# dblanm/gnn-manip

Hardware: AMD Instinct MI355X
Metric: rollout steps/sec (N particles, 10 MP steps, hidden=128) (higher is better)
Workload: dtype f32; 1 GPU; north_star target: N=100k dense synthetic scene, conn_r=0.015, max_neighbours=20, hidden=128, 10 MP steps; n_particles=100000, hidden=128, edges_last_step=1966056, k_steps=6, candidates_per_gpu=1, parallelism=candidate-parallel x1

## Files before the change

gnn_manip_amd/csrc/hedge.hip:

```cpp
#include <type_traits>
#include "common.h"
#include "mlp.h"
#include "hedge.h"
#include "hmlp.h"
#include "hmma_dev.h"
#include "blocks_dev.h"

namespace gm {

namespace {

constexpr int H = 128;
constexpr int BE = 32;
constexpr int SYS_THREADS = 768;
static_assert(BE == kBlockEdges, "block tables and the systolic kernels agree on the block size");
#ifdef HEDGE_STAMPS
__device__ unsigned long long g_sys_stamps[3 * 32 * 8 + 32];
#define SYS_STAMP(tick, slot)                                                                                         \
    do {                                                                                                              \
        if (blockIdx.x == 0 && jb == 0 && lane0 == 0 && (tick) >= 16 && (tick) < 48) {                                \
            g_sys_stamps[(role * 32 + (tick) - 16) * 8 + (slot)] = __builtin_readcyclecounter();                     \
            if (role == 0 && (slot) == 0) g_sys_stamps[3 * 32 * 8 + (tick) - 16] = __builtin_amdgcn_s_memrealtime(); \
        }                                                                                                             \
    } while (0)
// ... 141 lines not shown
}
__device__ __forceinline__ float sum_of_halves(float v) {
    const auto r = __builtin_amdgcn_permlane32_swap(__float_as_uint(v), __float_as_uint(v), false, false);
    return __uint_as_float(r[0]) + __uint_as_float(r[1]);
}

template <int R>
__device__ __forceinline__ void scan3_t(float& ya, float& yb, float& yc, float yprev, unsigned cont) {
    asm volatile("s_bfe_i32 exec_lo, %4, %5\n\ts_bfe_i32 exec_hi, %4, %6\n\tv_add_f32 %0, %0, %3\n\t"
                 "s_bfe_i32 exec_lo, %4, %7\n\ts_bfe_i32 exec_hi, %4, %8\n\tv_add_f32 %1, %1, %0\n\t"
                 "s_bfe_i32 exec_lo, %4, %9\n\ts_bfe_i32 exec_hi, %4, %10\n\tv_add_f32 %2, %2, %1\n\t"
                 "s_mov_b64 exec, -1"
                 : "+v"(ya), "+v"(yb), "+v"(yc)
                 : "v"(yprev), "s"(cont), "n"(0x10000 | R), "n"(0x10000 | (16 + R)), "n"(0x10000 | (R + 1)), "n"(0x10000 | (17 + R)),
                   "n"(0x10000 | (R + 2)), "n"(0x10000 | (18 + R))
                 : "scc");
}
__device__ __forceinline__ void scan3(float& ya, float& yb, float& yc, float yprev, unsigned cont, int r) {
    switch (r) {
        case 1: scan3_t<1>(ya, yb, yc, yprev, cont); break;
        case 4: scan3_t<4>(ya, yb, yc, yprev, cont); break;
        case 7: scan3_t<7>(ya, yb, yc, yprev, cont); break;
        case 10: scan3_t<10>(ya, yb, yc, yprev, cont); break;
        default: scan3_t<13>(ya, yb, yc, yprev, cont); break;
    }
}


__device__ __forceinline__ int2 wg_range(int units, bool xcd_major) {
    const int wg = xcd_major ? xcd_major_wg() : (int)blockIdx.x;
    return make_int2((int)((long long)wg * units / gridDim.x), (int)((long long)(wg + 1) * units / gridDim.x));
}

template <int NP, class I = int>
__device__ __forceinline__ void sys_prologue(half8 (&wh)[8], half8 (&wl)[8], const half8* frag, int slice, bool one_kgroup, int zero_end, int vec_b, const float* vec, int n_vec) {
    const int tid = threadIdx.x, lane0 = tid & 63;
#pragma unroll
    for (int ks = 0; ks < 8; ++ks) {
        const int kq = one_kgroup ? 0 : ks;
        wh[ks] = frag[(((I)slice * 8 + kq) * 2 + 0) * 64 + lane0];
        if constexpr (NP == 3) wl[ks] = frag[(((I)slice * 8 + kq) * 2 + 1) * 64 + lane0];
    }
    for (int i = tid; i < zero_end / 16; i += SYS_THREADS) LDS(uintx4, i * 16) = uintx4{0u, 0u, 0u, 0u};
    for (int i = tid; i < n_vec; i += SYS_THREADS) LDS(float, vec_b + 4 * i) = vec[i];
    __builtin_amdgcn_s_waitcnt(0x0f70);
    __syncthreads();
}

__device__ __forceinline__ void set_role_prio(int role) {
    if (role == 2) __builtin_amdgcn_s_setprio(3);
    else __builtin_amdgcn_s_setprio(1);
}

__device__ __forceinline__ floatx16 vec_to_acc(char* smem, int vec_b, int f, int jb, int hi) {
    floatx16 a;
#pragma unroll
    for (int g = 0; g < 4; ++g) {
        const floatx4 v = LDS(floatx4, vec_b + (f + 32 * jb + 4 * hi + 8 * g) * 4);
#pragma unroll
        for (int tt = 0; tt < 4; ++tt) a[4 * g + tt] = v[tt];
    }
    return a;
}

__device__ __forceinline__ void publish_ln_stats(const floatx16& acc, unsigned st_w, unsigned z_w) {
    float q = 0.f;
#pragma unroll
    for (int r = 0; r < 16; ++r) q = fmaf(acc[r], acc[r], q);
    LDS(float, st_w) = sum_of_halves(q);
#pragma unroll
    for (int g = 0; g < 4; ++g) {
        floatx4 z;
#pragma unroll
        for (int tt = 0; tt < 4; ++tt) z[tt] = acc[4 * g + tt];
        LDS(floatx4, z_w + 32 * g) = z;
    }
}

// ... 34 lines not shown
        if (nb & 1) {                                                                                \
            tick(int_c<0>{}, nb + 1);                                                                \
            tick_as(int_c<1>{}, int_c<TICK_DRAIN>{}, nb + 2);                                        \
        } else {                                                                                     \
            tick_as(int_c<0>{}, int_c<TICK_DRAIN>{}, nb + 2);                                        \
        }                                                                                            \
    }

template <bool MAY_BE_NULL = true>
__device__ __forceinline__ void report_split_range(int rng, int lane0, int* flags) {
    if (rng && lane0 == 0 && (!MAY_BE_NULL || flags)) atomicOr(flags, ERRF_SPLIT_RANGE);
}

template <bool WRITE_E, bool STREAM, int NP>
__global__ void __launch_bounds__(SYS_THREADS, 1) sys_edge_kernel(const CsrHeader* a_hdr, const int* __restrict__ a_dst, const int* __restrict__ a_src, const float* __restrict__ a_P,
                                                                       const float* a_e_in, float* a_e_out, float* __restrict__ a_agg, const float* __restrict__ a_hw,
                                                                       const int2* __restrict__ a_blk, const int2* __restrict__ a_seg, const int* __restrict__ a_head,
                                                                       const EdgeBlockHeader* __restrict__ a_tab, unsigned a_side_off, unsigned a_agg_bytes, unsigned a_P_bytes,
                                                                       int* a_flags, float a_eps, int a_residual) {
    const int tid = threadIdx.x, lane0 = tid & 63;
    const int wave = __builtin_amdgcn_readfirstlane(tid >> 6);
#ifdef HEDGE_FORCE_ROLE
    const int role = HEDGE_FORCE_ROLE, jb = wave & 3;
#else
    const int role = wave >> 2, jb = wave & 3;
#endif
    const int E = a_hdr->n_edges;
    const int2 cr = wg_range(a_tab->n_groups, true);
    if (cr.y <= cr.x) return;
    const int b0 = 4 * cr.x, b1 = 4 * cr.y;
    const int nb = b1 - b0;
    if (nb <= 0) return;
    const float inv_T = a_hw[1];
    half8 wh[8], wl[8];
    sys_prologue<NP>(wh, wl, reinterpret_cast<const half8*>(a_hw + HW_HEADER_FLOATS + HW_VEC_FLOATS), role * 4 + jb, false, L_ZERO_END, L_VEC,
                      a_hw + HW_HEADER_FLOATS, 4 * H);
    auto ok = [&](int x) { return x >= b0 && x < b1; };
    auto clampb = [&](int x) { return x < b0 ? b0 : (x < b1 ? x : b1 - 1); };
    const int e0 = a_blk[b0].x;
    const srd_t srd_ein = make_srd(a_e_in + (size_t)e0 * H, 0xffffffffu);
    const int n = lane0 & 31, hi = lane0 >> 5, rr = lane0 >> 3, cq = lane0 & 7;
    const unsigned v_eoff = opaque(rr * 512 + jb * 128 + cq * 16);
    set_role_prio(role);
    if (role == 0) {
        const srd_t srd_P = make_srd(a_P, a_P_bytes);
        const unsigned idx_bytes = (unsigned)s_clamp0(E - e0, 1 << 28) * 4u;
        const srd_t srd_dst = make_srd(a_dst + e0, idx_bytes), srd_src = make_srd(a_src + e0, idx_bytes);
        const unsigned v_poff = opaque(jb * 128 + cq * 16), v_ioff = opaque(rr * 16);
        const unsigned ps_w = opaque(L_PS + jb * TILE_B + 4 * rr * TILE_ROW_B + cq * 16);
        const unsigned ps_r = opaque(L_PS + jb * TILE_B + n * TILE_ROW_B + hi * 16);
        const int kg = cq & 1, ksb = cq >> 2, half = (cq >> 1) & 1;
        const unsigned e_w = opaque(L_E + ((2 * jb + ksb) * 2 * 64 + ((rr ^ (2 * (ksb + 2 * kg))) + 32 * kg)) * 16 + half * 8);
        const unsigned e_r0 = opaque(L_E + eslot(n, hi, 0) * 16), e_r1 = opaque(L_E + eslot(n, hi, 1) * 16);
        const unsigned x1_w = opaque(L_X1 + 4 * jb * 1024 + lane0 * 16);
        floatx4 pi[4], pj[4];
#pragma unroll
        for (int j = 0; j < 4; ++j) { pi[j] = floatx4{0.f, 0.f, 0.f, 0.f}; pj[j] = pi[j]; }
        int rng = 0;
        floatx4 eq[4];
#pragma unroll
        for (int j = 0; j < 4; ++j) eq[j] = bld4(srd_ein, v_eoff, j * 4096);
        floatx16 acc, c0v;
#pragma unroll
        for (int r = 0; r < 16; ++r) { c0v[r] = 0.f; acc[r] = 0.f; }
        intx4 di = bldi4(srd_dst, v_ioff, 0), si = bldi4(srd_src, v_ioff, 0);
        int2 be = a_blk[clampb(b0 + 1)];
        auto tick_as = [&](auto par_c, auto kind_c, int t) __attribute__((always_inline)) {
            constexpr int PAR = decltype(par_c)::value;
            constexpr int KIND = decltype(kind_c)::value;
            if constexpr (KIND == TICK_IDLE) {
                lds_barrier();
                return;
            }
            if constexpr (KIND == TICK_LAST) {
                auto nothing = [](int) {};
                mlp_layer<NP>(acc, c0v, wh, wl, smem, e_r0 + PAR * IMG_B, e_r1 + PAR * IMG_B, nothing);
                rng |= __any(row_bad<NP>(acc[0])) ? 1 : 0;
                GM_SB;
                acc_to_image<NP>(acc, smem, x1_w + PAR * IMG_B);
                lds_barrier();
                return;
            }
            const int x = b0 + t;
            SYS_STAMP(t, 0);
            auto prepare = [&]() {
#pragma unroll
                for (int j = 0; j < 4; ++j) LDS(floatx4, ps_w + j * TILE_ROW_B) = pi[j] + pj[j];
#pragma unroll
                for (int g = 0; g < 4; ++g) {
                    const floatx4 v = LDS(floatx4, ps_r + 32 * g);
#pragma unroll
                    for (int tt = 0; tt < 4; ++tt) c0v[4 * g + tt] = v[tt];
                }
            };
            SYS_STAMP(t, 1);
            if (jb == 0 && cq == 0) LDS(intx4, v_ioff + (L_DR + ((x + 1) & (DR_SLOTS - 1)) * (BE * 4))) = di;
            const unsigned rel = (unsigned)(be.x - e0);
            auto p_loads = [&](int j) {
// ... 20 lines not shown
                } else if (slot == 8) {
#pragma unroll
                    for (int j = 0; j < 4; ++j) eq[j] = bld4(srd_ein, v_eoff, rel * 512 + j * 4096);
                    be = be_next;
                }
            };
            SYS_STAMP(t, 2);
            if constexpr (KIND == TICK_FULL) {
                mlp_layer<NP>(acc, c0v, wh, wl, smem, e_r0 + PAR * IMG_B, e_r1 + PAR * IMG_B, side);
                SYS_STAMP(t, 3);
                rng |= __any(row_bad<NP>(acc[0])) ? 1 : 0;
                GM_SB;
                acc_to_image<NP>(acc, smem, x1_w + PAR * IMG_B);
            } else {
#pragma unroll
                for (int slot = 0; slot <= 8; ++slot) side(slot);
            }
            SYS_STAMP(t, 4);
            prepare();
            SYS_STAMP(t, 5);
            lds_barrier();
            SYS_STAMP(t, 6);
        };
        auto tick = [&](auto par_c, int t) __attribute__((always_inline)) { tick_as(par_c, int_c<TICK_FULL>{}, t); };
        tick_as(int_c<1>{}, int_c<TICK_FILL>{}, -1);
        tick(int_c<0>{}, tick_no(0));
        RUN_TICKS(1, nb - 3, tick);
        tick_as(int_c<1>{}, int_c<TICK_LAST>{}, nb - 1);
        tick_as(int_c<0>{}, int_c<TICK_IDLE>{}, nb);
        tick_as(int_c<1>{}, int_c<TICK_IDLE>{}, nb + 1);
        tick_as(int_c<0>{}, int_c<TICK_IDLE>{}, nb + 2);
        report_split_range<false>(rng, lane0, a_flags);
    } else if (role == 1) {
        floatx16 acc;
#pragma unroll
        for (int r = 0; r < 16; ++r) acc[r] = 0.f;
        int rng = 0;
        floatx4 er = floatx4{0.f, 0.f, 0.f, 0.f};
        int st_a = e0, cnt_a = 0, st_b = e0, cnt_b = 0;
        int2 bi_c = a_blk[b0];
        const float res_w = a_residual ? 1.f : 0.f;
        const floatx4 gm = LDS(floatx4, L_VEC + (2 * H + 32 * jb + 4 * cq) * 4);
        const floatx4 bt = LDS(floatx4, L_VEC + (3 * H + 32 * jb + 4 * cq) * 4);
        const floatx16 b2v = vec_to_acc(smem, L_VEC, 0, jb, hi);
        const unsigned st_r = opaque(L_ST + n * 4);
        const unsigned km_w = opaque(L_KM + jb * 128 + n * 4), km_r = opaque(L_KM + jb * 128 + rr * 4);
        const unsigned z_r = opaque(L_Z + jb * TILE_B + rr * TILE_ROW_B + cq * 16);
        const unsigned x_in = opaque(L_X1 + lane0 * 16), x_out = opaque(L_X2 + 4 * jb * 1024 + lane0 * 16);
        float* const e_out_wg = a_e_out + (size_t)e0 * H;
        auto tick_as = [&](auto par_c, auto kind_c, int t) {
            constexpr int PAR = decltype(par_c)::value, P1 = 1 - PAR, P3 = 1 - PAR;
            constexpr int KIND = decltype(kind_c)::value;
            const int x = b0 + t;
            if constexpr (KIND == TICK_IDLE) {
                const int2 bi_i = a_blk[clampb(x)];
                st_a = st_b; cnt_a = cnt_b;
                st_b = bi_c.x; cnt_b = bi_c.y & 0xff;
                bi_c = bi_i;
                lds_barrier();
                return;
            }
            SYS_STAMP(t, 0);
            if (WRITE_E) LDS(float, km_w) = ln_k(smem, st_r + P3 * 512, inv_T, a_eps);
            const int cnt_st = ok(x - 3) ? cnt_a : 0;
            const int2 bi_n = a_blk[clampb(x)];
            const unsigned rel_a = (unsigned)(st_a - e0), rel_b = (unsigned)(st_b - e0);
// ... 2 lines not shown
                if (!WRITE_E) return;
                if (slot == 0) lg.load(km_r, z_r + P3 * 4 * TILE_B);
                else if (slot == 2)
                    lg.store<STREAM ? ST_STREAM_E : 0>(e_out_wg, rel_a, 0, cnt_st, v_eoff, gm, bt, er, res_w, srd_ein, rel_b);
            };
            SYS_STAMP(t, 1);
            SYS_STAMP(t, 2);
            if constexpr (KIND == TICK_FULL) {
                mlp_layer<NP>(acc, b2v, wh, wl, smem, x_in + P1 * IMG_B, x_in + P1 * IMG_B, side);
                rng |= __any(row_bad<NP>(acc[0])) ? 1 : 0;
                GM_SB;
                acc_to_image<NP>(acc, smem, x_out + P1 * IMG_B);
            } else {
#pragma unroll
                for (int slot = 0; slot <= 2; ++slot) side(slot);
            }
            SYS_STAMP(t, 3);
            SYS_STAMP(t, 4);
            st_a = st_b; cnt_a = cnt_b;
            st_b = bi_c.x; cnt_b = bi_c.y & 0xff;
            bi_c = bi_n;
            SYS_STAMP(t, 5);
            lds_barrier();
            SYS_STAMP(t, 6);
        };
        auto tick = [&](auto par_c, int t) { tick_as(par_c, int_c<TICK_FULL>{}, t); };
        tick_as(int_c<1>{}, int_c<TICK_IDLE>{}, -1);
        tick_as(int_c<0>{}, int_c<TICK_IDLE>{}, 0);
        RUN_TICKS(1, nb - 1, tick);
        tick_as(int_c<1>{}, int_c<TICK_DRAIN>{}, nb + 1);
        tick_as(int_c<0>{}, int_c<TICK_DRAIN>{}, nb + 2);
        report_split_range<false>(rng, lane0, a_flags);
    } else {
        floatx16 acc;
        int rng = 0;
        float carry = 0.f;
        int cnt_a = 0, fl_a = 0, cnt_b = 0, fl_b = 0;
        unsigned cont_a = 0, last_a = 0, cont_b = 0, last_b = 0;
        int head_a = -1, head_b = -1;
        int2 bn = a_blk[b0], sn = make_int2(0, 0);
        const float gam = LDS(float, L_VEC + (2 * H + 32 * jb + n) * 4), bet = LDS(float, L_VEC + (3 * H + 32 * jb + n) * 4);
        const float res_w = a_residual ? 1.f : 0.f;
        floatx4 er[3];
#pragma unroll
        for (int j = 0; j < 3; ++j) er[j] = floatx4{0.f, 0.f, 0.f, 0.f};
        int st_a = e0, st_b = e0;
        const unsigned km_re = opaque(L_KM2 + jb * 128 + rr * 4);
        const unsigned z_e = opaque(L_Z + jb * TILE_B + rr * TILE_ROW_B + cq * 16);
        float* const e_out_wg = a_e_out + (size_t)e0 * H;
        const unsigned v_aoff = opaque(L_ST + jb * 128 + n * 4);
        const unsigned st_r = opaque(L_ST + n * 4);
        const unsigned km_rq = opaque(L_KM2 + jb * 128 + 64 * hi);
        const unsigned z_w = opaque(L_Z + jb * TILE_B + n * TILE_ROW_B + hi * 16);
        const unsigned z_t = opaque(L_Z + jb * TILE_B + 16 * hi * TILE_ROW_B + n * 4);
        const unsigned x_in = opaque(L_X2 + lane0 * 16);
        const unsigned dr_r = opaque(L_DR + 64 * hi);
        const srd_t srd_agg = make_srd(reinterpret_cast<const char*>(a_agg) - L_ST, a_agg_bytes + L_ST);
        floatx16 b3v = vec_to_acc(smem, L_VEC, H, jb, hi);
        auto fetch = [&](int x, int2 bi, int2 si, int hd, int& st, int& cnt, int& fl, unsigned& cont, unsigned& last, int& head) {
            st = bi.x;
            if (!ok(x)) { cnt = 0; fl = 0; cont = 0; last = 0; return; }
            cnt = bi.y & 0xff;
            fl = bi.y >> 8;
            cont = (unsigned)si.x;
            last = (unsigned)si.y;
            if (fl & 1) head = hd;
// ... 102 lines not shown
            }
            }
            SYS_STAMP(t, 4);
            stores();
            cnt_a = cnt_b; fl_a = fl_b; cont_a = cont_b; last_a = last_b;
            if (fl_b & 1) head_a = head_b;
            st_a = st_b;
            fetch(x - 1, bn, sn, hd_n, st_b, cnt_b, fl_b, cont_b, last_b, head_b);
            bn = bn_n;
            sn = sn_n;
            SYS_STAMP(t, 5);
            lds_barrier();
            SYS_STAMP(t, 6);
        };
        auto tick = [&](auto par_c, int t) __attribute__((always_inline)) { tick_as(par_c, int_c<TICK_FULL>{}, t); };
        tick_as(int_c<1>{}, int_c<TICK_IDLE>{}, -1);
        tick_as(int_c<0>{}, int_c<TICK_IDLE>{}, 0);
        tick_as(int_c<1>{}, int_c<TICK_IDLE>{}, 1);
        tick(int_c<0>{}, tick_no(2));
        RUN_TICKS(3, nb - 1, tick);
        tick(int_c<1>{}, nb + 1);
        tick_as(int_c<0>{}, int_c<TICK_DRAIN>{}, nb + 2);
        report_split_range<false>(rng, lane0, a_flags);
    }
}

constexpr int LE_X1 = 0;
constexpr int LE_X2 = LE_X1 + 2 * IMG_B;
constexpr int LE_Z = LE_X2 + 2 * IMG_B;
constexpr int LE_ST = LE_Z + 8 * TILE_B;
constexpr int LE_KM = LE_ST + 2 * 4 * 32 * 4;
constexpr int RS_SLOTS = 8;
constexpr int LE_RS = LE_KM + 4 * 32 * 4;
constexpr int LE_ZERO_END = LE_RS + RS_SLOTS * 32 * 4;
constexpr int LE_VEC = LE_ZERO_END;
constexpr size_t ENC_LDS_BYTES = LE_VEC + 5 * H * 4;

template <int NP>
__global__ void __launch_bounds__(SYS_THREADS, 1) sys_enc_kernel(const CsrHeader* a_hdr, const float* __restrict__ a_x, float* __restrict__ a_e_out,
                                                                      const float* __restrict__ a_hw, int* a_flags, float a_eps, int a_pad_rows) {
    const int tid = threadIdx.x, lane0 = tid & 63;
    const int wave = __builtin_amdgcn_readfirstlane(tid >> 6);
    const int role = wave >> 2, jb = wave & 3;
    const int E = a_hdr->n_edges;
    const int nblk = (E + BE - 1) / BE;
    const int2 br = wg_range(nblk, true);
    const int b0 = br.x, b1 = br.y;
    const int nb = b1 - b0;
    if (a_pad_rows && blockIdx.x == 0)
        for (int i = tid; i < kEdgePadRows * H / 4; i += SYS_THREADS) reinterpret_cast<floatx4*>(a_e_out + (size_t)E * H)[i] = floatx4{0.f, 0.f, 0.f, 0.f};
    if (nb <= 0) return;
    const float inv_T = a_hw[1], cap = a_hw[2];
    half8 wh[8], wl[8];
    sys_prologue<NP>(wh, wl, reinterpret_cast<const half8*>(a_hw + HW_HEADER_FLOATS + HW_VEC_FLOATS), role * 4 + jb, role == 0, LE_ZERO_END, LE_VEC,
                      a_hw + HW_HEADER_FLOATS, 5 * H);
    const int n = lane0 & 31, hi = lane0 >> 5, rr = lane0 >> 3, cq = lane0 & 7;
    const int e0 = b0 * BE;
    const int rows_wg = (b1 * BE < E ? b1 * BE : E) - e0;
    floatx16 bv;
    {
        const int slot = role == 0 ? 4 : role - 1;
#pragma unroll
        for (int g = 0; g < 4; ++g) {
            const floatx4 v = LDS(floatx4, LE_VEC + (slot * H + 32 * jb + 4 * hi + 8 * g) * 4);
#pragma unroll
            for (int tt = 0; tt < 4; ++tt) bv[4 * g + tt] = v[tt];
        }
    }
    const unsigned rs_l = opaque(LE_RS + n * 4);
    int rng = 0;
    floatx16 acc;
    auto scaled_bias = [&](float sc) {
        floatx16 c;
#pragma unroll
        for (int r = 0; r < 16; ++r) c[r] = bv[r] * sc;
        return c;
    };
    if (role == 0) {
        const srd_t srd_x = make_srd(a_x + (size_t)e0 * 4, (unsigned)(rows_wg > 0 ? rows_wg : 0) * 16u);
        float* const e_out_wg = a_e_out + (size_t)e0 * H;
        const unsigned v_xoff = opaque(n * 16 + (hi ? 0x40000000u : 0u));
        const unsigned v_eoff = opaque(rr * 512 + jb * 128 + cq * 16);
        const unsigned x1_w = opaque(LE_X1 + 4 * jb * 1024 + lane0 * 16);
        const unsigned st_r = opaque(LE_ST + n * 4);
        const unsigned km_w = opaque(LE_KM + jb * 128 + n * 4), km_r = opaque(LE_KM + jb * 128 + rr * 4);
        const unsigned z_r = opaque(LE_Z + jb * TILE_B + rr * TILE_ROW_B + cq * 16);
        const floatx4 gm = LDS(floatx4, LE_VEC + (2 * H + 32 * jb + 4 * cq) * 4);
        const floatx4 bt = LDS(floatx4, LE_VEC + (3 * H + 32 * jb + 4 * cq) * 4);
        const float T3 = 1.0f / inv_T;
        floatx4 xq = bld4(srd_x, v_xoff, 0);
        auto tick = [&](auto par_c, int t) {
            constexpr int PAR = decltype(par_c)::value, P3 = 1 - PAR;
            const int x = b0 + t;
            float mx = fmaxf(fmaxf(fabsf(xq[0]), fabsf(xq[1])), fmaxf(fabsf(xq[2]), fabsf(xq[3])));
            float sc = cap;
            if (mx > 0.f && mx < 3.0e38f) {
                int ex;
                (void)frexpf(mx, &ex);
                sc = fminf(ldexpf(1.f, min(7 - ex, 100)), cap);
            }
            sc = lower_half_to_both(sc);
            if (jb == 0 && hi == 0) LDS(float, rs_l + (x & (RS_SLOTS - 1)) * 128) = sc;
            uintx2 h, l;
            if constexpr (NP == 3) split4(xq[0] * sc, xq[1] * sc, xq[2] * sc, xq[3] * sc, h, l);
            else hi4(xq[0] * sc, xq[1] * sc, xq[2] * sc, xq[3] * sc, h);
            const half8 bh = __builtin_bit_cast(half8, uintx4{h[0], h[1], 0u, 0u});
            const floatx16 c0v = scaled_bias(sc);
            {
                const int xn = x + 1 < b0 ? b0 : (x + 1 < b1 ? x + 1 : b1 - 1);
                xq = bld4(srd_x, v_xoff, (unsigned)(xn - b0) * 512u);
            }
            if constexpr (NP == 3) {
            const half8 bl = __builtin_bit_cast(half8, uintx4{l[0], l[1], 0u, 0u});
            acc = __builtin_amdgcn_mfma_f32_32x32x16_f16(wl[0], bh, c0v, 0, 0, 0);
            acc = __builtin_amdgcn_mfma_f32_32x32x16_f16(wh[0], bl, acc, 0, 0, 0);
            acc = __builtin_amdgcn_mfma_f32_32x32x16_f16(wh[0], bh, acc, 0, 0, 0);
            } else {
                acc = __builtin_amdgcn_mfma_f32_32x32x16_f16(wh[0], bh, c0v, 0, 0, 0);
            }
            {
                const float rs3 = LDS(float, rs_l + ((x - 3) & (RS_SLOTS - 1)) * 128);
                const float q = (LDS(float, st_r + P3 * 512) + LDS(float, st_r + P3 * 512 + 128)) + (LDS(float, st_r + P3 * 512 + 256) + LDS(float, st_r + P3 * 512 + 384));
                const float tt3 = T3 * rs3;
                const float v = fmaf(a_eps * tt3, tt3, q * (1.0f / 128.0f));
                float r = __builtin_amdgcn_rsqf(v);
                r = r * fmaf(-0.5f * v * r, r, 1.5f);
                LDS(float, km_w) = r;
                const int xb = x - 3;
                const int cnt = (xb >= b0 && xb < b1) ? min(BE, E - xb * BE) : 0;
#pragma unroll
                for (int j = 0; j < 4; ++j) {
                    const float kr = LDS(float, km_r + j * 32);
                    const floatx4 zq = LDS(floatx4, z_r + P3 * 4 * TILE_B + j * 8 * TILE_ROW_B);
                    floatx4 o;
#pragma unroll
                    for (int tt = 0; tt < 4; ++tt) o[tt] = fmaf(zq[tt] * kr, gm[tt], bt[tt]);
                    bst4s<ST_ENC_E>(make_srd(e_out_wg + (size_t)((xb - b0) * BE + 8 * j) * H, (unsigned)s_clamp0(cnt - 8 * j, 8) * 512u), v_eoff, 0, o);
                }
            }
            rng |= __any(row_bad<NP>(acc[0])) ? 1 : 0;
            GM_SB;
            acc_to_image<NP>(acc, smem, x1_w + PAR * IMG_B);
            lds_barrier();
        };
        RUN_TICKS(0, nb + 2, tick);
    } else if (role == 1) {
        const unsigned x_in = opaque(LE_X1 + lane0 * 16), x_out = opaque(LE_X2 + 4 * jb * 1024 + lane0 * 16);
        auto nothing = [](int) {};
        auto tick = [&](auto par_c, int t) {
            constexpr int PAR = decltype(par_c)::value, P1 = 1 - PAR;
            const int x = b0 + t;
            const floatx16 c0v = scaled_bias(LDS(float, rs_l + ((x - 1) & (RS_SLOTS - 1)) * 128));
            mlp_layer<NP>(acc, c0v, wh, wl, smem, x_in + P1 * IMG_B, x_in + P1 * IMG_B, nothing);
            rng |= __any(row_bad<NP>(acc[0])) ? 1 : 0;
            GM_SB;
            acc_to_image<NP>(acc, smem, x_out + P1 * IMG_B);
            lds_barrier();
        };
        RUN_TICKS(0, nb + 2, tick);
    } else {
        const unsigned x_in = opaque(LE_X2 + lane0 * 16);
        const unsigned st_w = opaque(LE_ST + jb * 128 + n * 4);
        const unsigned z_w = opaque(LE_Z + jb * TILE_B + n * TILE_ROW_B + hi * 16);
        auto nothing = [](int) {};
        auto tick = [&](auto par_c, int t) {
            constexpr int PAR = decltype(par_c)::value, P2 = PAR;
            const int x = b0 + t;
            const floatx16 c0v = scaled_bias(LDS(float, rs_l + ((x - 2) & (RS_SLOTS - 1)) * 128));
            mlp_layer<NP>(acc, c0v, wh, wl, smem, x_in + P2 * IMG_B, x_in + P2 * IMG_B, nothing);
            rng |= __any(row_bad<NP>(acc[0])) ? 1 : 0;
            publish_ln_stats(acc, st_w + P2 * 512, z_w + P2 * 4 * TILE_B);
            lds_barrier();
        };
        RUN_TICKS(0, nb + 2, tick);
    }
    report_split_range(rng, lane0, a_flags);
}

constexpr int LN_E = 0;
constexpr int LN_X1 = LN_E + 2 * IMG_B;
constexpr int LN_X2 = LN_X1 + 2 * IMG_B;
constexpr int LN_Z = LN_X2 + 2 * IMG_B;
constexpr int LN_PS = LN_Z + 8 * TILE_B;
constexpr int LN_ST = LN_PS + 4 * TILE_B;
constexpr int LN_KM = LN_ST + 2 * 4 * 32 * 4;
constexpr int LN_ZERO_END = LN_KM + 2 * 4 * 32 * 4;
constexpr int LN_VEC = LN_ZERO_END;
constexpr size_t NODE_LDS_BYTES = LN_VEC + 4 * H * 4;
static_assert(NODE_LDS_BYTES <= 160 * 1024, "LDS budget");

template <int NP>
__device__ __forceinline__ void sys_node_body(const float* a_h, const float* __restrict__ a_agg, const float* __restrict__ a_Q,
                                              float* a_h_out, const float* __restrict__ a_hw, int a_n, int* a_flags, float a_eps) {
    const int tid = threadIdx.x, lane0 = tid & 63;
    const int wave = __builtin_amdgcn_readfirstlane(tid >> 6);
    const int role = wave >> 2, jb = wave & 3;
    const int N = a_n;
    const int nblk = (N + BE - 1) / BE;
    const int wg = (int)blockIdx.x;
    const int b0 = (int)((long long)wg * nblk / gridDim.x), b1 = (int)((long long)(wg + 1) * nblk / gridDim.x);
    const int nb = b1 - b0;
    if (nb <= 0) return;
    const float inv_T = a_hw[1];
    half8 wh[8], wl[8];
    sys_prologue<NP>(wh, wl, reinterpret_cast<const half8*>(a_hw + HW_HEADER_FLOATS + HW_VEC_FLOATS), role * 4 + jb, false, LN_ZERO_END, LN_VEC,
                 a_hw + HW_HEADER_FLOATS, 4 * H);
    const int n = lane0 & 31, hi = lane0 >> 5, rr = lane0 >> 3, cq = lane0 & 7;
    const int r0 = b0 * BE;
    const int rows_wg = (b1 * BE < N ? b1 * BE : N) - r0;
    const unsigned wg_bytes = (unsigned)(rows_wg > 0 ? rows_wg : 0) * 512u;
    const unsigned v_eoff = opaque(rr * 512 + jb * 128 + cq * 16);
    int rng = 0;
    set_role_prio(role);
    if (role == 0) {
        const srd_t srd_q = make_srd(a_Q + (size_t)r0 * H, wg_bytes), srd_a = make_srd(a_agg + (size_t)r0 * H, wg_bytes);
        const unsigned v_qoff = opaque(rr * 2048 + jb * 128 + cq * 16);
        const unsigned ps_w = opaque(LN_PS + jb * TILE_B + 4 * rr * TILE_ROW_B + cq * 16);
        const unsigned ps_r = opaque(LN_PS + jb * TILE_B + n * TILE_ROW_B + hi * 16);
        const int kg = cq & 1, ksb = cq >> 2, half = (cq >> 1) & 1;
        const unsigned e_w = opaque(LN_E + ((2 * jb + ksb) * 2 * 64 + ((rr ^ (2 * (ksb + 2 * kg))) + 32 * kg)) * 16 + half * 8);
        const unsigned e_r0 = opaque(LN_E + eslot(n, hi, 0) * 16), e_r1 = opaque(LN_E + eslot(n, hi, 1) * 16);
        const unsigned x1_w = opaque(LN_X1 + 4 * jb * 1024 + lane0 * 16);
        floatx4 qv[4], eq[4];
#pragma unroll
        for (int j = 0; j < 4; ++j) { qv[j] = floatx4{0.f, 0.f, 0.f, 0.f}; eq[j] = bld4(srd_a, v_eoff, j * 4096); }
        floatx16 acc, c0v;
#pragma unroll
        for (int r = 0; r < 16; ++r) c0v[r] = 0.f;
        auto clampb = [&](int x) { return x < b0 ? b0 : (x < b1 ? x : b1 - 1); };
        auto tick_as = [&](auto par_c, auto kind_c, int t) {
            constexpr int PAR = decltype(par_c)::value, KIND = decltype(kind_c)::value;
            if constexpr (KIND == TICK_DRAIN) {
                lds_barrier();
                return;
            }
            const int x = b0 + t;
            const unsigned rel1 = (unsigned)(clampb(x + 1) - b0) * (BE * 512u), rel2 = (unsigned)(clampb(x + 2) - b0) * (BE * 512u);
#pragma unroll
            for (int j = 0; j < 4; ++j) qv[j] = bld4(srd_q, v_qoff, rel1 + j * 512);
            auto side = [&](int slot) {
                if (slot < 8 && !(slot & 1)) {
                    const int j = slot >> 1;
                    uintx2 h, l;
                    if constexpr (NP == 3) split4(eq[j][0], eq[j][1], eq[j][2], eq[j][3], h, l);
                    else hi4(eq[j][0], eq[j][1], eq[j][2], eq[j][3], h);
                    LDS(uintx2, e_w + (1 - PAR) * IMG_B + j * 128) = h;
                    if constexpr (NP == 3) LDS(uintx2, e_w + (1 - PAR) * IMG_B + j * 128 + 1024) = l;
                } else if (slot == 8) {
#pragma unroll
                    for (int j = 0; j < 4; ++j) eq[j] = bld4(srd_a, v_eoff, rel2 + j * 4096);
                }
            };
            if constexpr (KIND == TICK_FULL) {
                mlp_layer<NP>(acc, c0v, wh, wl, smem, e_r0 + PAR * IMG_B, e_r1 + PAR * IMG_B, side);
                rng |= __any(row_bad<NP>(acc[0])) ? 1 : 0;
                GM_SB;
                acc_to_image<NP>(acc, smem, x1_w + PAR * IMG_B);
            } else {
#pragma unroll
                for (int slot = 0; slot <= 8; ++slot) side(slot);
            }
#pragma unroll
            for (int j = 0; j < 4; ++j) LDS(floatx4, ps_w + j * TILE_ROW_B) = qv[j];
#pragma unroll
            for (int g = 0; g < 4; ++g) {
                const floatx4 v = LDS(floatx4, ps_r + 32 * g);
#pragma unroll
                for (int tt = 0; tt < 4; ++tt) c0v[4 * g + tt] = v[tt];
            }
            lds_barrier();
        };
        NODE_TICKS(tick_as);
    } else {
        const bool r2 = role == 2;
        const int eg0 = r2 ? 2 : 0;
        const srd_t srd_h = make_srd(a_h + (size_t)r0 * H, wg_bytes);
        float* const h_out_wg = a_h_out + (size_t)r0 * H;
        const floatx4 gm = LDS(floatx4, LN_VEC + (2 * H + 32 * jb + 4 * cq) * 4);
        const floatx4 bt = LDS(floatx4, LN_VEC + (3 * H + 32 * jb + 4 * cq) * 4);
        const floatx16 bv = vec_to_acc(smem, LN_VEC, r2 ? H : 0, jb, hi);
        const unsigned st_r = opaque(LN_ST + n * 4);
        const unsigned km_w = opaque(LN_KM + (r2 ? 512 : 0) + jb * 128 + n * 4), km_r = opaque(LN_KM + (r2 ? 512 : 0) + jb * 128 + rr * 4);
        const unsigned z_r = opaque(LN_Z + jb * TILE_B + rr * TILE_ROW_B + cq * 16);
        const unsigned x_in = opaque((r2 ? LN_X2 : LN_X1) + lane0 * 16), x_out = opaque(LN_X2 + 4 * jb * 1024 + lane0 * 16);
        const unsigned st_w = opaque(LN_ST + jb * 128 + n * 4);
        const unsigned z_w = opaque(LN_Z + jb * TILE_B + n * TILE_ROW_B + hi * 16);
        floatx4 er[2];
        er[0] = er[1] = floatx4{0.f, 0.f, 0.f, 0.f};
        floatx16 acc;
        auto tick_as = [&](auto par_c, auto kind_c, int t) {
            constexpr int PAR = decltype(par_c)::value, PIN = 1 - PAR, P3 = 1 - PAR;
            constexpr int KIND = decltype(kind_c)::value;
            if constexpr (KIND == TICK_FILL) {
                lds_barrier();
                return;
            }
            const int x = b0 + t;
            LDS(float, km_w) = ln_k(smem, st_r + P3 * 512, inv_T, a_eps);
            const int xb = x - 3;
            const int cnt = (xb >= b0 && xb < b1) ? min(BE, N - xb * BE) : 0;
            const unsigned rel_a = (unsigned)((xb < b0 ? b0 : xb) - b0) * BE;
            const int xr = x - 2 < b0 ? b0 : (x - 2 < b1 ? x - 2 : b1 - 1);
            const unsigned rel_b = (unsigned)(xr - b0) * (BE * 512u);
            float kr;
            floatx4 zq;
            auto side = [&](int slot) {
// ... 34 lines not shown
__global__ void __launch_bounds__(SYS_THREADS, 1) sys_node_kernel(const float* a_h, const float* __restrict__ a_agg, const float* __restrict__ a_Q,
                                                                       float* a_h_out, const float* __restrict__ a_hw, int a_n, int* a_flags, float a_eps) {
    sys_node_body<NP>(a_h, a_agg, a_Q, a_h_out, a_hw, a_n, a_flags, a_eps);
}

constexpr int LP_E = 0;
constexpr int LP_T = LP_E + 2 * IMG_B;
constexpr size_t PROJ_LDS_BYTES = LP_T + 12 * TILE_B;

template <int LD_H, int NP>
__device__ __forceinline__ void sys_proj_body(const float* __restrict__ a_h, float* __restrict__ a_P, float* __restrict__ a_Q,
                                              const float* __restrict__ a_wp, const float* __restrict__ a_wq,
                                              const float* __restrict__ a_sp, const float* __restrict__ a_sq, int a_n, int* a_flags) {
    const int tid = threadIdx.x, lane0 = tid & 63;
    const int wave = __builtin_amdgcn_readfirstlane(tid >> 6);
    const int N = a_n;
    const int nblk = (N + BE - 1) / BE;
    const int b0 = (int)((long long)blockIdx.x * nblk / gridDim.x), b1 = (int)((long long)(blockIdx.x + 1) * nblk / gridDim.x);
    const int nb = b1 - b0;
    if (nb <= 0) return;
    const bool isq = wave >= 8;
    const float* img = isq ? a_wq : a_wp;
    const int ob = isq ? wave - 8 : wave;
    const int out_pad = isq ? H : 2 * H;
    const float out_scale = img[1] * (isq ? (a_sq ? *a_sq : 1.f) : (a_sp ? *a_sp : 1.f));
    const int n = lane0 & 31, hi = lane0 >> 5, rr = lane0 >> 3, cq = lane0 & 7;
    floatx16 bv;
#pragma unroll
    for (int g = 0; g < 4; ++g) {
        const floatx4 v = *reinterpret_cast<const floatx4*>(img + 4 + 32 * ob + 8 * g + 4 * hi);
#pragma unroll
        for (int tt = 0; tt < 4; ++tt) bv[4 * g + tt] = v[tt];
    }
    half8 wh[8], wl[8];
    sys_prologue<NP, size_t>(wh, wl, reinterpret_cast<const half8*>(img + 4 + out_pad), ob, false, LP_E + 2 * IMG_B, 0, nullptr, 0);
    const int r0 = b0 * BE;
    const int rows_wg = (b1 * BE < N ? b1 * BE : N) - r0;
    const unsigned wg_bytes = (unsigned)(rows_wg > 0 ? rows_wg : 0) * 512u;
    const srd_t srd_h = make_srd(a_h + (size_t)r0 * H, wg_bytes);
    const bool producer = wave < 8;
    unsigned v_in[2], e_w[2];
#pragma unroll
    for (int i = 0; i < 2; ++i) {
        const int u = 2 * (wave & 7) + i, j = u >> 2, sb = u & 3;
        const int kg = cq & 1, ksb = cq >> 2, half = (cq >> 1) & 1;
        v_in[i] = opaque((unsigned)((8 * j + rr) * 512 + sb * 128 + cq * 16));
        e_w[i] = opaque((unsigned)(LP_E + ((2 * sb + ksb) * 2 * 64 + ((rr ^ (2 * (ksb + 2 * kg))) + 32 * kg)) * 16 + half * 8 + j * 128));
    }
    const unsigned e_r0 = opaque(LP_E + eslot(n, hi, 0) * 16), e_r1 = opaque(LP_E + eslot(n, hi, 1) * 16);
    const unsigned t_w = opaque(LP_T + wave * TILE_B + n * TILE_ROW_B + hi * 16);
    const unsigned t_r = opaque(LP_T + wave * TILE_B + rr * TILE_ROW_B + cq * 16);
    float* const out_wg = isq ? a_Q + (size_t)r0 * H + 32 * ob : a_P + (size_t)r0 * 2 * H + 32 * ob;
    const unsigned out_row_b = isq ? 512u : 1024u;
    const unsigned v_out = opaque((unsigned)(rr * out_row_b + cq * 16));
    auto clampb = [&](int x) { return x < b0 ? b0 : (x < b1 ? x : b1 - 1); };
    floatx4 hq[2];
#pragma unroll
    for (int i = 0; i < 2; ++i) hq[i] = producer ? bld4s<LD_H>(srd_h, v_in[i], 0) : floatx4{0.f, 0.f, 0.f, 0.f};
    int rng = 0;
    floatx16 acc;
    auto tick_as = [&](auto par_c, auto kind_c, int t) {
        constexpr int PAR = decltype(par_c)::value, KIND = decltype(kind_c)::value;
        const int x = b0 + t;
        const unsigned rel2 = (unsigned)(clampb(x + 2) - b0) * (BE * 512u);
        const int cnt = (x >= b0 && x < b1) ? min(BE, N - x * BE) : 0;
        auto side = [&](int slot) {
            if (producer && (slot == 0 || slot == 2)) {
                const int i = slot >> 1;
                uintx2 h, l;
                if constexpr (NP == 3) split4(hq[i][0], hq[i][1], hq[i][2], hq[i][3], h, l);
                else hi4(hq[i][0], hq[i][1], hq[i][2], hq[i][3], h);
                LDS(uintx2, e_w[i] + (1 - PAR) * IMG_B) = h;
                if constexpr (NP == 3) LDS(uintx2, e_w[i] + (1 - PAR) * IMG_B + 1024) = l;
            } else if (producer && slot == 4) {
#pragma unroll
                for (int i = 0; i < 2; ++i) hq[i] = bld4s<LD_H>(srd_h, v_in[i], rel2);
            }
        };
        if constexpr (KIND == TICK_FILL) {
#pragma unroll
            for (int slot = 0; slot <= 4; ++slot) side(slot);
            lds_barrier();
            return;
        }
        mlp_layer<NP>(acc, bv, wh, wl, smem, e_r0 + PAR * IMG_B, e_r1 + PAR * IMG_B, side);
        rng |= __any(row_bad<NP>(acc[0])) ? 1 : 0;
#pragma unroll
        for (int g = 0; g < 4; ++g) {
            floatx4 z;
// ... 371 lines not shown
```

Before: 127.8 rollout steps/s.

## Overlap systolic kernel prologues with first global loads and trim LDS zeroing

The shared prologue now issues each role's first global loads (edge features, indices, node Q/agg rows, encoder inputs) before the LDS zeroing and barrier, so that load latency hides behind setup. LDS zeroing is limited to the ranges that actually need it instead of the whole prefix, and the vector constants go through registers. The edge encoder gets explicit fill, steady and drain ticks per role, so dead epilogue work and dummy ticks at pipeline start and end are skipped. The risk is a barrier-count mismatch between roles or LDS regions that are no longer zeroed but are still read.

After: 128.0 rollout steps/s (median of 6 runs). About the same (+0.2%).

```diff
diff --git a/gnn_manip_amd/csrc/hedge.hip b/gnn_manip_amd/csrc/hedge.hip
--- a/gnn_manip_amd/csrc/hedge.hip
+++ b/gnn_manip_amd/csrc/hedge.hip
@@ -197,8 +197,13 @@
     return make_int2((int)((long long)wg * units / gridDim.x), (int)((long long)(wg + 1) * units / gridDim.x));
 }
 
-template <int NP, class I = int>
-__device__ __forceinline__ void sys_prologue(half8 (&wh)[8], half8 (&wl)[8], const half8* frag, int slice, bool one_kgroup, int zero_end, int vec_b, const float* vec, int n_vec) {
+struct LdsZero {
+    int b0, e0, b1, e1, b2, e2;
+};
+
+template <int NP, class I = int, class F>
+__device__ __forceinline__ void sys_prologue(half8 (&wh)[8], half8 (&wl)[8], const half8* frag, int slice, bool one_kgroup, const LdsZero zero, int vec_b, const float* vec, int n_vec,
+                                             F&& first_requests) {
     const int tid = threadIdx.x, lane0 = tid & 63;
 #pragma unroll
     for (int ks = 0; ks < 8; ++ks) {
@@ -206,9 +211,14 @@
         wh[ks] = frag[(((I)slice * 8 + kq) * 2 + 0) * 64 + lane0];
         if constexpr (NP == 3) wl[ks] = frag[(((I)slice * 8 + kq) * 2 + 1) * 64 + lane0];
     }
-    for (int i = tid; i < zero_end / 16; i += SYS_THREADS) LDS(uintx4, i * 16) = uintx4{0u, 0u, 0u, 0u};
-    for (int i = tid; i < n_vec; i += SYS_THREADS) LDS(float, vec_b + 4 * i) = vec[i];
+    float vv = 0.f;
+    if (tid < n_vec) vv = vec[tid];
+    first_requests();
+    for (int i = zero.b0 / 16 + tid; i < zero.e0 / 16; i += SYS_THREADS) LDS(uintx4, i * 16) = uintx4{0u, 0u, 0u, 0u};
+    for (int i = zero.b1 / 16 + tid; i < zero.e1 / 16; i += SYS_THREADS) LDS(uintx4, i * 16) = uintx4{0u, 0u, 0u, 0u};
+    for (int i = zero.b2 / 16 + tid; i < zero.e2 / 16; i += SYS_THREADS) LDS(uintx4, i * 16) = uintx4{0u, 0u, 0u, 0u};
     __builtin_amdgcn_s_waitcnt(0x0f70);
+    if (tid < n_vec) LDS(float, vec_b + 4 * tid) = vv;
     __syncthreads();
 }
 
@@ -309,16 +319,18 @@
     const int nb = b1 - b0;
     if (nb <= 0) return;
     const float inv_T = a_hw[1];
-    half8 wh[8], wl[8];
-    sys_prologue<NP>(wh, wl, reinterpret_cast<const half8*>(a_hw + HW_HEADER_FLOATS + HW_VEC_FLOATS), role * 4 + jb, false, L_ZERO_END, L_VEC,
-                      a_hw + HW_HEADER_FLOATS, 4 * H);
     auto ok = [&](int x) { return x >= b0 && x < b1; };
     auto clampb = [&](int x) { return x < b0 ? b0 : (x < b1 ? x : b1 - 1); };
     const int e0 = a_blk[b0].x;
     const srd_t srd_ein = make_srd(a_e_in + (size_t)e0 * H, 0xffffffffu);
     const int n = lane0 & 31, hi = lane0 >> 5, rr = lane0 >> 3, cq = lane0 & 7;
     const unsigned v_eoff = opaque(rr * 512 + jb * 128 + cq * 16);
-    set_role_prio(role);
+    half8 wh[8], wl[8];
+    auto prologue = [&](auto&& first_requests) __attribute__((always_inline)) {
+        sys_prologue<NP>(wh, wl, reinterpret_cast<const half8*>(a_hw + HW_HEADER_FLOATS + HW_VEC_FLOATS), role * 4 + jb, false,
+                         LdsZero{L_Z, L_PS, L_ST, L_ZERO_END, 0, 0}, L_VEC, a_hw + HW_HEADER_FLOATS, 4 * H, first_requests);
+        set_role_prio(role);
+    };
     if (role == 0) {
         const srd_t srd_P = make_srd(a_P, a_P_bytes);
         const unsigned idx_bytes = (unsigned)s_clamp0(E - e0, 1 << 28) * 4u;
@@ -335,12 +347,16 @@
         for (int j = 0; j < 4; ++j) { pi[j] = floatx4{0.f, 0.f, 0.f, 0.f}; pj[j] = pi[j]; }
         int rng = 0;
         floatx4 eq[4];
-#pragma unroll
-        for (int j = 0; j < 4; ++j) eq[j] = bld4(srd_ein, v_eoff, j * 4096);
+        intx4 di, si;
+        prologue([&]() {
+#pragma unroll
+            for (int j = 0; j < 4; ++j) eq[j] = bld4(srd_ein, v_eoff, j * 4096);
+            di = bldi4(srd_dst, v_ioff, 0);
+            si = bldi4(srd_src, v_ioff, 0);
+        });
         floatx16 acc, c0v;
 #pragma unroll
         for (int r = 0; r < 16; ++r) { c0v[r] = 0.f; acc[r] = 0.f; }
-        intx4 di = bldi4(srd_dst, v_ioff, 0), si = bldi4(srd_src, v_ioff, 0);
         int2 be = a_blk[clampb(b0 + 1)];
         auto tick_as = [&](auto par_c, auto kind_c, int t) __attribute__((always_inline)) {
             constexpr int PAR = decltype(par_c)::value;
@@ -427,6 +443,7 @@
         tick_as(int_c<0>{}, int_c<TICK_IDLE>{}, nb + 2);
         report_split_range<false>(rng, lane0, a_flags);
     } else if (role == 1) {
+        prologue([]() {});
         floatx16 acc;
 #pragma unroll
         for (int r = 0; r < 16; ++r) acc[r] = 0.f;
@@ -495,6 +512,7 @@
         tick_as(int_c<0>{}, int_c<TICK_DRAIN>{}, nb + 2);
         report_split_range<false>(rng, lane0, a_flags);
     } else {
+        prologue([]() {});
         floatx16 acc;
         int rng = 0;
         float carry = 0.f;
@@ -663,8 +681,7 @@
 constexpr int LE_KM = LE_ST + 2 * 4 * 32 * 4;
 constexpr int RS_SLOTS = 8;
 constexpr int LE_RS = LE_KM + 4 * 32 * 4;
-constexpr int LE_ZERO_END = LE_RS + RS_SLOTS * 32 * 4;
-constexpr int LE_VEC = LE_ZERO_END;
+constexpr int LE_VEC = LE_RS + RS_SLOTS * 32 * 4;
 constexpr size_t ENC_LDS_BYTES = LE_VEC + 5 * H * 4;
 
 template <int NP>
@@ -682,12 +699,17 @@
         for (int i = tid; i < kEdgePadRows * H / 4; i += SYS_THREADS) reinterpret_cast<floatx4*>(a_e_out + (size_t)E * H)[i] = floatx4{0.f, 0.f, 0.f, 0.f};
     if (nb <= 0) return;
     const float inv_T = a_hw[1], cap = a_hw[2];
-    half8 wh[8], wl[8];
-    sys_prologue<NP>(wh, wl, reinterpret_cast<const half8*>(a_hw + HW_HEADER_FLOATS + HW_VEC_FLOATS), role * 4 + jb, role == 0, LE_ZERO_END, LE_VEC,
-                      a_hw + HW_HEADER_FLOATS, 5 * H);
     const int n = lane0 & 31, hi = lane0 >> 5, rr = lane0 >> 3, cq = lane0 & 7;
     const int e0 = b0 * BE;
     const int rows_wg = (b1 * BE < E ? b1 * BE : E) - e0;
+    half8 wh[8], wl[8];
+    floatx4 xq = floatx4{0.f, 0.f, 0.f, 0.f};
+    const srd_t srd_x = make_srd(a_x + (size_t)e0 * 4, (unsigned)(rows_wg > 0 ? rows_wg : 0) * 16u);
+    const unsigned v_xoff = opaque(n * 16 + (hi ? 0x40000000u : 0u));
+    sys_prologue<NP>(wh, wl, reinterpret_cast<const half8*>(a_hw + HW_HEADER_FLOATS + HW_VEC_FLOATS), role * 4 + jb, role == 0, LdsZero{0, 0, 0, 0, 0, 0}, LE_VEC,
+                     a_hw + HW_HEADER_FLOATS, 5 * H, [&]() {
+                         if (role == 0) xq = bld4(srd_x, v_xoff, 0);
+                     });
     floatx16 bv;
     {
         const int slot = role == 0 ? 4 : role - 1;
@@ -708,9 +730,7 @@
         return c;
     };
     if (role == 0) {
-        const srd_t srd_x = make_srd(a_x + (size_t)e0 * 4, (unsigned)(rows_wg > 0 ? rows_wg : 0) * 16u);
         float* const e_out_wg = a_e_out + (size_t)e0 * H;
-        const unsigned v_xoff = opaque(n * 16 + (hi ? 0x40000000u : 0u));
         const unsigned v_eoff = opaque(rr * 512 + jb * 128 + cq * 16);
         const unsigned x1_w = opaque(LE_X1 + 4 * jb * 1024 + lane0 * 16);
         const unsigned st_r = opaque(LE_ST + n * 4);
@@ -719,10 +739,38 @@
         const floatx4 gm = LDS(floatx4, LE_VEC + (2 * H + 32 * jb + 4 * cq) * 4);
         const floatx4 bt = LDS(floatx4, LE_VEC + (3 * H + 32 * jb + 4 * cq) * 4);
         const float T3 = 1.0f / inv_T;
-        floatx4 xq = bld4(srd_x, v_xoff, 0);
-        auto tick = [&](auto par_c, int t) {
-            constexpr int PAR = decltype(par_c)::value, P3 = 1 - PAR;
+        auto tick_as = [&](auto par_c, auto kind_c, int t) {
+            constexpr int PAR = decltype(par_c)::value, P3 = 1 - PAR, KIND = decltype(kind_c)::value;
+            if constexpr (KIND == TICK_IDLE) {
+                lds_barrier();
+                return;
+            }
             const int x = b0 + t;
+            auto epilogue = [&]() {
+                const float rs3 = LDS(float, rs_l + ((x - 3) & (RS_SLOTS - 1)) * 128);
+                const float q = (LDS(float, st_r + P3 * 512) + LDS(float, st_r + P3 * 512 + 128)) + (LDS(float, st_r + P3 * 512 + 256) + LDS(float, st_r + P3 * 512 + 384));
+                const float tt3 = T3 * rs3;
+                const float v = fmaf(a_eps * tt3, tt3, q * (1.0f / 128.0f));
+                float r = __builtin_amdgcn_rsqf(v);
+                r = r * fmaf(-0.5f * v * r, r, 1.5f);
+                LDS(float, km_w) = r;
+                const int xb = x - 3;
+                const int cnt = (xb >= b0 && xb < b1) ? min(BE, E - xb * BE) : 0;
+#pragma unroll
+                for (int j = 0; j < 4; ++j) {
+                    const float kr = LDS(float, km_r + j * 32);
+                    const floatx4 zq = LDS(floatx4, z_r + P3 * 4 * TILE_B + j * 8 * TILE_ROW_B);
+                    floatx4 o;
+#pragma unroll
+                    for (int tt = 0; tt < 4; ++tt) o[tt] = fmaf(zq[tt] * kr, gm[tt], bt[tt]);
+                    bst4s<ST_ENC_E>(make_srd(e_out_wg + (size_t)((xb - b0) * BE + 8 * j) * H, (unsigned)s_clamp0(cnt - 8 * j, 8) * 512u), v_eoff, 0, o);
+                }
+            };
+            if constexpr (KIND == TICK_DRAIN) {
+                epilogue();
+                lds_barrier();
+                return;
+            }
             float mx = fmaxf(fmaxf(fabsf(xq[0]), fabsf(xq[1])), fmaxf(fabsf(xq[2]), fabsf(xq[3])));
             float sc = cap;
             if (mx > 0.f && mx < 3.0e38f) {
@@ -749,32 +797,35 @@
             } else {
                 acc = __builtin_amdgcn_mfma_f32_32x32x16_f16(wh[0], bh, c0v, 0, 0, 0);
             }
-            {
-                const float rs3 = LDS(float, rs_l + ((x - 3) & (RS_SLOTS - 1)) * 128);
-                const float q = (LDS(float, st_r + P3 * 512) + LDS(float, st_r + P3 * 512 + 128)) + (LDS(float, st_r + P3 * 512 + 256) + LDS(float, st_r + P3 * 512 + 384));
-                const float tt3 = T3 * rs3;
-                const float v = fmaf(a_eps * tt3, tt3, q * (1.0f / 128.0f));
-                float r = __builtin_amdgcn_rsqf(v);
-                r = r * fmaf(-0.5f * v * r, r, 1.5f);
-                LDS(float, km_w) = r;
-                const int xb = x - 3;
-                const int cnt = (xb >= b0 && xb < b1) ? min(BE, E - xb * BE) : 0;
-#pragma unroll
-                for (int j = 0; j < 4; ++j) {
-                    const float kr = LDS(float, km_r + j * 32);
-                    const floatx4 zq = LDS(floatx4, z_r + P3 * 4 * TILE_B + j * 8 * TILE_ROW_B);
-                    floatx4 o;
-#pragma unroll
-                    for (int tt = 0; tt < 4; ++tt) o[tt] = fmaf(zq[tt] * kr, gm[tt], bt[tt]);
-                    bst4s<ST_ENC_E>(make_srd(e_out_wg + (size_t)((xb - b0) * BE + 8 * j) * H, (unsigned)s_clamp0(cnt - 8 * j, 8) * 512u), v_eoff, 0, o);
-                }
-            }
+            if constexpr (KIND == TICK_FULL) epilogue();
             rng |= __any(row_bad<NP>(acc[0])) ? 1 : 0;
             GM_SB;
             acc_to_image<NP>(acc, smem, x1_w + PAR * IMG_B);
             lds_barrier();
         };
-        RUN_TICKS(0, nb + 2, tick);
+        auto tick = [&](auto par_c, int t) { tick_as(par_c, int_c<TICK_FULL>{}, t); };
+        auto fill = [&](auto par_c, int t) {
+            if (t < nb) tick_as(par_c, int_c<TICK_FILL>{}, t);
+            else tick_as(par_c, int_c<TICK_IDLE>{}, t);
+        };
+        auto drain = [&](auto par_c, int t) {
+            if (t <= nb + 2) tick_as(par_c, int_c<TICK_DRAIN>{}, t);
+        };
+        fill(int_c<0>{}, 0);
+        fill(int_c<1>{}, 1);
+        fill(int_c<0>{}, 2);
+        RUN_TICKS(3, nb - 2, tick);
+        if (nb > 3 && !(nb & 1)) tick(int_c<1>{}, nb - 1);
+        const int td = nb > 3 ? nb : 3;
+        if (td & 1) {
+            drain(int_c<1>{}, td);
+            drain(int_c<0>{}, td + 1);
+            drain(int_c<1>{}, td + 2);
+        } else {
+            drain(int_c<0>{}, td);
+            drain(int_c<1>{}, td + 1);
+            drain(int_c<0>{}, td + 2);
+        }
     } else if (role == 1) {
         const unsigned x_in = opaque(LE_X1 + lane0 * 16), x_out = opaque(LE_X2 + 4 * jb * 1024 + lane0 * 16);
         auto nothing = [](int) {};
@@ -788,7 +839,11 @@
             acc_to_image<NP>(acc, smem, x_out + P1 * IMG_B);
             lds_barrier();
         };
-        RUN_TICKS(0, nb + 2, tick);
+        lds_barrier();
+        RUN_TICKS(1, nb - 1, tick);
+        if (nb & 1) tick(int_c<1>{}, nb);
+        lds_barrier();
+        lds_barrier();
     } else {
         const unsigned x_in = opaque(LE_X2 + lane0 * 16);
         const unsigned st_w = opaque(LE_ST + jb * 128 + n * 4);
@@ -803,7 +858,11 @@
             publish_ln_stats(acc, st_w + P2 * 512, z_w + P2 * 4 * TILE_B);
             lds_barrier();
         };
-        RUN_TICKS(0, nb + 2, tick);
+        lds_barrier();
+        lds_barrier();
+        RUN_TICKS(2, nb, tick);
+        if (nb & 1) tick(int_c<0>{}, nb + 1);
+        lds_barrier();
     }
     report_split_range(rng, lane0, a_flags);
 }
@@ -833,16 +892,18 @@
     const int nb = b1 - b0;
     if (nb <= 0) return;
     const float inv_T = a_hw[1];
-    half8 wh[8], wl[8];
-    sys_prologue<NP>(wh, wl, reinterpret_cast<const half8*>(a_hw + HW_HEADER_FLOATS + HW_VEC_FLOATS), role * 4 + jb, false, LN_ZERO_END, LN_VEC,
-                 a_hw + HW_HEADER_FLOATS, 4 * H);
     const int n = lane0 & 31, hi = lane0 >> 5, rr = lane0 >> 3, cq = lane0 & 7;
     const int r0 = b0 * BE;
     const int rows_wg = (b1 * BE < N ? b1 * BE : N) - r0;
     const unsigned wg_bytes = (unsigned)(rows_wg > 0 ? rows_wg : 0) * 512u;
     const unsigned v_eoff = opaque(rr * 512 + jb * 128 + cq * 16);
+    half8 wh[8], wl[8];
+    auto prologue = [&](auto&& first_requests) __attribute__((always_inline)) {
+        sys_prologue<NP>(wh, wl, reinterpret_cast<const half8*>(a_hw + HW_HEADER_FLOATS + HW_VEC_FLOATS), role * 4 + jb, false,
+                         LdsZero{LN_X1 + IMG_B, LN_X2 + IMG_B, LN_Z, LN_PS, LN_ST, LN_ZERO_END}, LN_VEC, a_hw + HW_HEADER_FLOATS, 4 * H, first_requests);
+        set_role_prio(role);
+    };
     int rng = 0;
-    set_role_prio(role);
     if (role == 0) {
         const srd_t srd_q = make_srd(a_Q + (size_t)r0 * H, wg_bytes), srd_a = make_srd(a_agg + (size_t)r0 * H, wg_bytes);
         const unsigned v_qoff = opaque(rr * 2048 + jb * 128 + cq * 16);
@@ -853,8 +914,12 @@
         const unsigned e_r0 = opaque(LN_E + eslot(n, hi, 0) * 16), e_r1 = opaque(LN_E + eslot(n, hi, 1) * 16);
         const unsigned x1_w = opaque(LN_X1 + 4 * jb * 1024 + lane0 * 16);
         floatx4 qv[4], eq[4];
-#pragma unroll
-        for (int j = 0; j < 4; ++j) { qv[j] = floatx4{0.f, 0.f, 0.f, 0.f}; eq[j] = bld4(srd_a, v_eoff, j * 4096); }
+        prologue([&]() {
+#pragma unroll
+            for (int j = 0; j < 4; ++j) eq[j] = bld4(srd_a, v_eoff, j * 4096);
+#pragma unroll
+            for (int j = 0; j < 4; ++j) qv[j] = bld4(srd_q, v_qoff, j * 512);
+        });
         floatx16 acc, c0v;
 #pragma unroll
         for (int r = 0; r < 16; ++r) c0v[r] = 0.f;
@@ -867,8 +932,10 @@
             }
             const int x = b0 + t;
             const unsigned rel1 = (unsigned)(clampb(x + 1) - b0) * (BE * 512u), rel2 = (unsigned)(clampb(x + 2) - b0) * (BE * 512u);
-#pragma unroll
-            for (int j = 0; j < 4; ++j) qv[j] = bld4(srd_q, v_qoff, rel1 + j * 512);
+            if constexpr (KIND != TICK_FILL) {
+#pragma unroll
+                for (int j = 0; j < 4; ++j) qv[j] = bld4(srd_q, v_qoff, rel1 + j * 512);
+            }
             auto side = [&](int slot) {
                 if (slot < 8 && !(slot & 1)) {
                     const int j = slot >> 1;
@@ -903,6 +970,7 @@
         };
         NODE_TICKS(tick_as);
     } else {
+        prologue([]() {});
         const bool r2 = role == 2;
         const int eg0 = r2 ? 2 : 0;
         const srd_t srd_h = make_srd(a_h + (size_t)r0 * H, wg_bytes);
@@ -1003,8 +1071,6 @@
 #pragma unroll
         for (int tt = 0; tt < 4; ++tt) bv[4 * g + tt] = v[tt];
     }
-    half8 wh[8], wl[8];
-    sys_prologue<NP, size_t>(wh, wl, reinterpret_cast<const half8*>(img + 4 + out_pad), ob, false, LP_E + 2 * IMG_B, 0, nullptr, 0);
     const int r0 = b0 * BE;
     const int rows_wg = (b1 * BE < N ? b1 * BE : N) - r0;
     const unsigned wg_bytes = (unsigned)(rows_wg > 0 ? rows_wg : 0) * 512u;
@@ -1026,6 +1092,8 @@
     const unsigned v_out = opaque((unsigned)(rr * out_row_b + cq * 16));
     auto clampb = [&](int x) { return x < b0 ? b0 : (x < b1 ? x : b1 - 1); };
     floatx4 hq[2];
+    half8 wh[8], wl[8];
+    sys_prologue<NP, size_t>(wh, wl, reinterpret_cast<const half8*>(img + 4 + out_pad), ob, false, LdsZero{LP_E, LP_E + 2 * IMG_B, 0, 0, 0, 0}, 0, nullptr, 0, []() {});
 #pragma unroll
     for (int i = 0; i < 2; ++i) hq[i] = producer ? bld4s<LD_H>(srd_h, v_in[i], 0) : floatx4{0.f, 0.f, 0.f, 0.f};
     int rng = 0;
```
